# danilobellini/audiolazy

Measured on NVIDIA H100. Metric: samples/sec through 64-ch gammatone bank, higher is better.
Workload: dtype f64

## Files before the change

### audiolazy_b200/csrc/alz_capi.cu

```cuda
#pragma GCC visibility push(default)
#include "../../include/alz_b200.h"
#pragma GCC visibility pop
#include "alz_biquad.cuh"
#include "alz_generic.cuh"
#include "alz_lane_tma.cuh"
#include "alz_plan.h"

#include <algorithm>
#include <cctype>
#include <cmath>
#include <cstring>
#include <map>
#include <thread>

#include <sys/mman.h>
#include <sys/syscall.h>
#include <unistd.h>

static std::mutex g_host_mu;
static std::map<void*, size_t> g_host_allocs;

static_assert(ALZI_OK == ALZ_OK && ALZI_ERR_CUDA == ALZ_ERR_CUDA && ALZI_ERR_UNSUPPORTED == ALZ_ERR_UNSUPPORTED, "status codes");

static thread_local std::string g_err;
// ... 101 lines not shown
    const cuuint64_t ystr[3] = {(cuuint64_t)ta.T * 4, (cuuint64_t)ta.ys * 4, (cuuint64_t)ta.ysS * 4};
    const cuuint32_t ybox[4] = {32, 32, 1, 1};
    return enc(tmy, CU_TENSOR_MAP_DATA_TYPE_FLOAT32, 4, (void*)ta.y, ydims, ystr, ybox, estr, CU_TENSOR_MAP_INTERLEAVE_NONE,
               CU_TENSOR_MAP_SWIZZLE_128B, CU_TENSOR_MAP_L2_PROMOTION_NONE, CU_TENSOR_MAP_FLOAT_OOB_FILL_NONE) == CUDA_SUCCESS;
  }
  {
    const cuuint64_t dims[3] = {(cuuint64_t)ta.T, (cuuint64_t)ta.S, 1};
    const cuuint64_t strides[2] = {(cuuint64_t)ta.xs * 4, (cuuint64_t)ta.xs * 4};
    const cuuint32_t box[3] = {32, 32, 1};
    if (enc(tmx, CU_TENSOR_MAP_DATA_TYPE_FLOAT32, 3, (void*)ta.x, dims, strides, box, estr, CU_TENSOR_MAP_INTERLEAVE_NONE,
            CU_TENSOR_MAP_SWIZZLE_128B, CU_TENSOR_MAP_L2_PROMOTION_L2_128B, CU_TENSOR_MAP_FLOAT_OOB_FILL_NONE) != CUDA_SUCCESS)
      return false;
  }
  {
    const cuuint64_t dims[4] = {(cuuint64_t)ta.T, (cuuint64_t)ta.C, (cuuint64_t)ta.S, 1};
    const cuuint64_t strides[3] = {(cuuint64_t)ta.ys * 4, (cuuint64_t)ta.ysS * 4, (cuuint64_t)ta.ysS * 4};
    const cuuint32_t box[4] = {32, 1, 32, 1};
    if (enc(tmy, CU_TENSOR_MAP_DATA_TYPE_FLOAT32, 4, (void*)ta.y, dims, strides, box, estr, CU_TENSOR_MAP_INTERLEAVE_NONE,
            CU_TENSOR_MAP_SWIZZLE_128B, CU_TENSOR_MAP_L2_PROMOTION_NONE, CU_TENSOR_MAP_FLOAT_OOB_FILL_NONE) != CUDA_SUCCESS)
      return false;
  }
  return true;
}

static bool make_map_2d(const float* ptr, long long T, long long n_rows, long long stride, CUtensorMap* tm) {
  alz_encode_tiled_fn enc = get_encode_tiled();
  if (!enc || ((uintptr_t)ptr & 15) || (stride & 3) || T >= (1ll << 31) || n_rows >= (1ll << 31)) return false;
  const cuuint32_t estr[2] = {1, 1};
  const cuuint64_t dims[2] = {(cuuint64_t)T, (cuuint64_t)n_rows};
  const cuuint64_t strides[1] = {(cuuint64_t)stride * 4};
  const cuuint32_t box[2] = {32, 32};
  return enc(tm, CU_TENSOR_MAP_DATA_TYPE_FLOAT32, 2, (void*)ptr, dims, strides, box, estr, CU_TENSOR_MAP_INTERLEAVE_NONE,
             CU_TENSOR_MAP_SWIZZLE_128B, CU_TENSOR_MAP_L2_PROMOTION_L2_128B, CU_TENSOR_MAP_FLOAT_OOB_FILL_NONE) == CUDA_SUCCESS;
}

static int launch_biquad(const alz_plan* p, const AlzTileArgs& ta, cudaStream_t st) {
  if (p->NB0 == 8) {
    if (p->K == 1) return alzi_launch_headfir_k1(p, ta, st);
    if (p->K == 4) return alzi_launch_headfir_k4(p, ta, st);
    return fail(ALZ_ERR_UNSUPPORTED, "no head-FIR kernel for K=%d", p->K);
  }
  switch (p->K) {
    case 1: return alzi_launch_biquad_k1(p, ta, st);
    case 2: return alzi_launch_biquad_k2(p, ta, st);
    case 3: return alzi_launch_biquad_k3(p, ta, st);
    case 4: return alzi_launch_biquad_k4(p, ta, st);
    case 6: return alzi_launch_biquad_k6(p, ta, st);
    case 8: return alzi_launch_biquad_k8(p, ta, st);
  }
  return fail(ALZ_ERR_UNSUPPORTED, "no biquad kernel for K=%d", p->K);
}

static double probe_biquad(const alz_plan* p, const double* r64, const double* r32) {
  if (p->NB0 == 8) return p->K == 1 ? alzi_probe_headfir_k1(p, r64, r32) : alzi_probe_headfir_k4(p, r64, r32);
  switch (p->K) {
    case 1: return alzi_probe_biquad_k1(p, r64, r32);
    case 2: return alzi_probe_biquad_k2(p, r64, r32);
    case 3: return alzi_probe_biquad_k3(p, r64, r32);
    case 4: return alzi_probe_biquad_k4(p, r64, r32);
    case 6: return alzi_probe_biquad_k6(p, r64, r32);
    default: return alzi_probe_biquad_k8(p, r64, r32);
  }
}

static int launch_generic(const alz_plan* p, AlzTileArgs ta, cudaStream_t st, const double* tv = nullptr,
                          long long tv_stride = 0) {
  AlzGenericArgs ga{p->d_sec, p->d_tap_delay, p->d_coef, p->K, p->C, 0, tv, tv_stride};
  const long long groups = (ta.S + 31) / 32;
  CUtensorMap tmx, tmy;
  if (alzi_make_tensor_maps(ta, &tmx, &tmy))
    alz_generic_tma_kernel<<<dim3((unsigned)p->C, (unsigned)groups), 32, ALZ_TMA_SMEM, st>>>(ta, ga, tmx, tmy);
  else
    alz_generic_kernel<<<dim3((unsigned)p->C, (unsigned)groups), 32, ALZ_WARP_SMEM, st>>>(ta, ga);
  ALZ_CUDA(cudaGetLastError());
  g_launches.fetch_add(1, std::memory_order_relaxed);
  return ALZ_OK;
}

static const int kBiquadKs[] = {1, 2, 3, 4, 6, 8};

extern "C" {

const char* alz_last_error(void) { return g_err.c_str(); }
int32_t alz_abi_version(void) { return ALZ_ABI_VERSION; }
int64_t alz_launch_count(void) { return g_launches.load(); }

int32_t alz_device_count(void) {
  int n = 0;
  if (cudaGetDeviceCount(&n) != cudaSuccess) { cudaGetLastError(); return 0; }
  return n;
}

int32_t alz_set_device(int32_t device) {
  ALZ_CUDA(cudaSetDevice(device));
  return ALZ_OK;
}

int32_t alz_plan_create(const double* coef, const int32_t* desc, int32_t C, int32_t KM, alz_plan** out) {
  return alz_plan_create_ex(coef, desc, C, KM, 0, out);
}

int32_t alz_plan_create_ex(const double* coef, const int32_t* desc, int32_t C, int32_t KM, int32_t flags,
                           alz_plan** out) {
  if (!out) return fail(ALZ_ERR_INVALID, "out is null");
  *out = nullptr;
  if (!coef || !desc || C <= 0 || KM < 0) return fail(ALZ_ERR_INVALID, "bad plan arguments");
  const bool design_only = (flags & ALZ_PLAN_DESIGN_ONLY) != 0;
  int dev = -1;
  if (!design_only) ALZ_CUDA(cudaGetDevice(&dev));

  struct Sec { std::vector<double> b, a; };
  std::vector<std::vector<Sec>> secs(C);
  int Kmax = 0, nbmax = 1, namax = 1;
  for (int c = 0; c < C; ++c) {
    bool ended = false;
    for (int k = 0; k < KM; ++k) {
      const int32_t* d = desc + ((size_t)c * KM + k) * 3;
      const int nb = d[0], na = d[1];
      if (nb == 0) { ended = true; continue; }
      if (ended) return fail(ALZ_ERR_INVALID, "channel %d: section %d follows an absent section", c, k);
      if (nb < 0 || na < 1 || d[2] < 0) return fail(ALZ_ERR_INVALID, "channel %d section %d: bad descriptor", c, k);
      const double* b = coef + d[2];
      const double* a = b + nb;
      if (a[0] == 0.0) return fail(ALZ_ERR_ZERO_GAIN, "channel %d section %d: Invalid filter gain (a0 == 0)", c, k);
      Sec s;
      s.b.assign(b, b + nb);
      s.a.assign(a, a + na);
      const double a0 = a[0];
      if (a0 != 1.0) {
        for (auto& v : s.b) v /= a0;
        for (auto& v : s.a) v /= a0;
        s.a[0] = 1.0;
      }
      while (s.b.size() > 1 && s.b.back() == 0.0) s.b.pop_back();
      while (s.a.size() > 1 && s.a.back() == 0.0) s.a.pop_back();
      for (double v : s.b) if (!std::isfinite(v)) return fail(ALZ_ERR_INVALID, "non-finite coefficient");
      for (double v : s.a) if (!std::isfinite(v)) return fail(ALZ_ERR_INVALID, "non-finite coefficient");
      nbmax = std::max(nbmax, (int)s.b.size());
      namax = std::max(namax, (int)s.a.size());
      secs[c].push_back(std::move(s));
    }
    Kmax = std::max(Kmax, (int)secs[c].size());
  }
  if (Kmax == 0) Kmax = 1;

  alz_plan* p = new (std::nothrow) alz_plan();
  if (!p) return fail(ALZ_ERR_NOMEM, "out of host memory");
  p->C = C;
  p->device = dev;
  p->sequential = (flags & ALZ_PLAN_SEQUENTIAL) != 0;
  p->parallel_sum = (flags & ALZ_PLAN_PARALLEL) != 0;
  if (design_only || cudaDeviceGetAttribute(&p->sm_count, cudaDevAttrMultiProcessorCount, dev) != cudaSuccess || p->sm_count <= 0) {
    cudaGetLastError();
    p->sm_count = 132;
  }

  p->fr_desc.assign((size_t)C * Kmax * 3, 0);
  for (int c = 0; c < C; ++c)
    for (size_t k = 0; k < secs[c].size(); ++k) {
      int* d = &p->fr_desc[((size_t)c * Kmax + k) * 3];
      d[0] = (int)secs[c][k].b.size(); d[1] = (int)secs[c][k].a.size(); d[2] = (int)p->fr_coef.size();
      p->fr_coef.insert(p->fr_coef.end(), secs[c][k].b.begin(), secs[c][k].b.end());
      p->fr_coef.insert(p->fr_coef.end(), secs[c][k].a.begin(), secs[c][k].a.end());
    }
  p->fr_K = Kmax;

  int nb_first = 1, nb_rest = 1;
  for (int c = 0; c < C; ++c)
    for (size_t k = 0; k < secs[c].size(); ++k) {
      if (k == 0) nb_first = std::max(nb_first, (int)secs[c][k].b.size());
      else nb_rest = std::max(nb_rest, (int)secs[c][k].b.size());
    }
  const bool plain = nbmax <= 3 && namax <= 3 && Kmax <= 8;
  const bool headfir = !plain && namax <= 3 && nb_first <= 8 && nb_rest <= 3 && Kmax <= 4;
  const bool biquad = (plain || headfir) && !(flags & ALZ_PLAN_FORCE_GENERIC);
  if (biquad) {
    int K = 8;
    for (int kk : kBiquadKs) if (kk >= Kmax) { K = kk; break; }
    if (headfir) K = Kmax == 1 ? 1 : 4;
    p->kind = ALZ_KIND_BIQUAD;
    p->K = K;
    p->NB = headfir ? (nb_rest <= 1 ? 1 : 3) : nbmax;
    p->NB0 = headfir ? 8 : 0;
    p->xd = ALZ_H0(p->NB0); p->yd = 2;
    p->state_doubles = ALZ_STATE_SLOTS(K, p->NB0);
    bool monic = !p->parallel_sum;
    for (int c = 0; c < C && monic; ++c) {
      double g = 1.0;
      for (auto& s : secs[c]) {
        const double b0 = s.b[0];
        if (!(std::fabs(b0) > 1e-150 && std::fabs(b0) < 1e150)) { monic = false; break; }
        g *= b0;
        if (!(std::fabs(g) > 1e-250 && std::fabs(g) < 1e250)) { monic = false; break; }
      }
    }
    bool gain_in = monic && !env_int("ALZ_EXACT_GAIN", 0);
    for (int c = 0; c < C && gain_in; ++c) {
      double g = 1.0;
      for (auto& s : secs[c]) g *= s.b[0];
      if (!(std::fabs(g) > 1e-30 && std::fabs(g) < 1e30)) gain_in = false;
    }
    p->monic = monic ? (gain_in ? 2 : 1) : 0;
    p->fp64_ops = (monic ? K * (p->NB - 1 + 2) + (gain_in ? 0 : 1) : K * (p->NB + 2)) + (headfir ? 8 - p->NB : 0);
    if (!headfir && !env_int("ALZ_NO_ZMASK", 0)) {
      int zm = (1 << (2 * K)) - 1;
      for (int c = 0; c < C; ++c)
        for (size_t k = 0; k < secs[c].size(); ++k)
          for (int j = 1; j <= 2; ++j)
            if ((int)secs[c][k].b.size() > j && secs[c][k].b[j] != 0.0) zm &= ~(1 << (2 * (int)k + j - 1));
      p->zmask = zm;
      if (K == 4 && p->NB == 3 && (zm & ALZ_ZMASK_KLAPURI) == ALZ_ZMASK_KLAPURI) p->fp64_ops -= 6;
    }
    const int stride = ALZ_COEF_STRIDE(K, p->NB0), nval = ALZ_COEF_NVAL(K, p->NB0);
    std::vector<double> tab((size_t)C * stride, 0.0);
    p->sc.assign((size_t)C * (K + 1), 1.0);
    for (int c = 0; c < C; ++c) {
      double* rec = tab.data() + (size_t)c * stride;
      double g = 1.0, sc = 1.0;
      if (p->monic == 2) {
        double gg = 1.0;
        for (auto& s : secs[c]) gg *= s.b[0];
        sc = (double)(float)gg;
        p->sc[(size_t)c * (K + 1)] = sc;
      }
      for (int k = 0; k < K; ++k) {
        double b[8] = {1.0, 0, 0, 0, 0, 0, 0, 0}, a[3] = {1.0, 0.0, 0.0};
        if (k < (int)secs[c].size()) {
          const Sec& s = secs[c][k];
          b[0] = 0.0;
          for (size_t i = 0; i < s.b.size(); ++i) b[i] = s.b[i];
          for (size_t i = 0; i < s.a.size(); ++i) a[i] = s.a[i];
        }
        if (k == 0 && p->NB0 == 8)
          for (int j = 3; j < 8; ++j) rec[5 * K + 1 + (j - 3)] = monic ? b[j] / b[0] : b[j];
        if (monic) {
          rec[5 * k + 0] = 1.0;
          rec[5 * k + 1] = b[1] / b[0];
          rec[5 * k + 2] = b[2] / b[0];
          g *= b[0];
          sc /= b[0];
        } else {
          rec[5 * k + 0] = b[0];
          rec[5 * k + 1] = b[1];
          rec[5 * k + 2] = b[2];
        }
        rec[5 * k + 3] = -a[1];
        rec[5 * k + 4] = -a[2];
        p->sc[(size_t)c * (K + 1) + k + 1] = sc;
      }
      rec[5 * K] = monic ? g : 1.0;
    }
    p->tier.assign(C, 0);
    p->tier_err.assign(C, -1.0);
    p->tier_tol = env_double("ALZ_TIER_TOL", 2.5e-6);
    p->probe_len = std::max(64, env_int("ALZ_TIER_PROBE", 8192));
    const bool tiering = !(flags & ALZ_PLAN_EXACT) && !p->parallel_sum && !env_int("ALZ_NO_FP32_TIER", 0) && p->tier_tol > 0.0;
    std::vector<double> tab32((size_t)C * stride, 0.0);
    for (int c = 0; c < C; ++c) {
      const double* rec = tab.data() + (size_t)c * stride;
      float* r32 = reinterpret_cast<float*>(tab32.data() + (size_t)c * stride);
      bool representable = true;
      for (int i = 0; i < nval; ++i) {
        r32[i] = (float)rec[i];
        if (rec[i] != 0.0 && !(std::fabs(rec[i]) > 1e-30 && std::fabs(rec[i]) < 1e30)) representable = false;
      }
      if (tiering && representable) {
        p->tier_err[c] = probe_biquad(p, rec, tab32.data() + (size_t)c * stride);
        if (p->tier_err[c] <= p->tier_tol) { p->tier[c] = 1; ++p->n_fp32; }
      }
    }
    {
      std::vector<int> lst[2];
      const int order = env_int("ALZ_TIER_ORDER", 1);
      for (int c = 0; c < C; ++c) lst[order == 1 ? p->tier[c] : (order == 2 ? 1 - p->tier[c] : 0)].push_back(c);
      size_t i0 = 0, i1 = 0;
      p->pos_channel.clear();
      while (i0 < lst[0].size() || i1 < lst[1].size()) {
        const bool take0 = i1 >= lst[1].size() || (i0 < lst[0].size() && i0 * lst[1].size() <= i1 * lst[0].size());
        p->pos_channel.push_back(take0 ? lst[0][i0++] : lst[1][i1++]);
      }
    }
    p->h_tab.assign((size_t)C * stride, 0.0);
    for (int pos = 0; pos < C; ++pos) {
      const int c = p->pos_channel[pos];
      const std::vector<double>& src = p->tier[c] ? tab32 : tab;
      double* rec = p->h_tab.data() + (size_t)pos * stride;
      memcpy(rec, src.data() + (size_t)c * stride, (size_t)nval * sizeof(double));
      rec[ALZ_COEF_META(K, p->NB0)] = (double)(c + 65536 * p->tier[c]);
    }
    p->fp64_ops_exact = p->fp64_ops;
    p->coef_small = C * stride <= kCoefSmall;
    const int ncoef = p->coef_small ? kCoefSmall : kCoefLarge;
    const int per_launch = ncoef / stride;
    if (per_launch < 1) { alz_plan_destroy(p); return fail(ALZ_ERR_UNSUPPORTED, "coefficient record too large"); }
    for (int p0 = 0; p0 < C; p0 += per_launch) {
      const int npos = std::min(per_launch, C - p0);
      char* blk = (char*)calloc(1, 2 * sizeof(int) + (size_t)ncoef * sizeof(double));
      if (!blk) { alz_plan_destroy(p); return fail(ALZ_ERR_NOMEM, "out of host memory"); }
      reinterpret_cast<int*>(blk)[0] = stride;
      reinterpret_cast<int*>(blk)[1] = npos;
      memcpy(blk + 2 * sizeof(int), p->h_tab.data() + (size_t)p0 * stride, (size_t)npos * stride * sizeof(double));
      p->chunks.push_back({blk, npos});
    }
    p->tile_group = env_int("ALZ_TILE_GROUP", 2);
    if (p->tile_group != 1 && p->tile_group != 2 && p->tile_group != 4) p->tile_group = 2;
  } else if (Kmax == 1 && !(flags & ALZ_PLAN_FORCE_GENERIC) && C * 32 <= kCoefLarge && !env_int("ALZ_NO_WINDOW", 0)) {
    p->kind = ALZ_KIND_GENERIC;
    p->window = true;
    p->K = 1;
    p->NB = nbmax;
    p->monic = 0;
    int near_x = 0, near_y = 0, maxd_x = 0, maxd_y = 0;
    std::vector<int> far_x, far_y;
    for (int c = 0; c < C; ++c) {
      if (secs[c].empty()) continue;
      const Sec& s = secs[c][0];
      for (size_t d = 1; d < s.b.size(); ++d)
        if (s.b[d] != 0.0) {
          maxd_x = std::max(maxd_x, (int)d);
          if (d < 16) near_x = std::max(near_x, (int)d);
          else if (std::find(far_x.begin(), far_x.end(), (int)d) == far_x.end()) far_x.push_back((int)d);
        }
      for (size_t d = 1; d < s.a.size(); ++d)
        if (s.a[d] != 0.0) {
          maxd_y = std::max(maxd_y, (int)d);
          if (d < 16) near_y = std::max(near_y, (int)d);
          else if (std::find(far_y.begin(), far_y.end(), (int)d) == far_y.end()) far_y.push_back((int)d);
        }
    }
    std::sort(far_x.begin(), far_x.end());
    std::sort(far_y.begin(), far_y.end());
    auto slots_of = [](int nearest) { return nearest == 0 ? 0 : (nearest <= 3 ? 4 : 16); };
    auto pow2 = [](int n) { int q = 1; while (q < n) q <<= 1; return q; };
    p->win_mx = slots_of(near_x);
    p->win_my = slots_of(near_y);
    p->win_nfx = (int)far_x.size();
    p->win_nfy = (int)far_y.size();
    int slot = 1;
    p->win_xwin = slot; slot += p->win_mx ? p->win_mx - 1 : 0;
    p->win_ywin = slot; slot += p->win_my ? p->win_my - 1 : 0;
    if (!far_x.empty()) { p->win_xbase = slot; p->win_xmask = pow2(far_x.back() + 16) - 1; slot += p->win_xmask + 1; }
    if (!far_y.empty()) { p->win_ybase = slot; p->win_ymask = pow2(far_y.back() + 16) - 1; slot += p->win_ymask + 1; }
    p->xd = maxd_x; p->yd = maxd_y;
    p->state_doubles = slot;
    p->fp64_ops = 1 + (p->win_mx ? p->win_mx - 1 : 0) + (p->win_my ? p->win_my - 1 : 0) + p->win_nfx + p->win_nfy;
    p->win_far_delay = far_x;
    p->win_far_delay.insert(p->win_far_delay.end(), far_y.begin(), far_y.end());
    p->h_tab.assign((size_t)C * 32, 0.0);
    std::vector<double> fcoef(std::max<size_t>(1, p->win_far_delay.size()) * C, 0.0);
    for (int c = 0; c < C; ++c) {
      double* rec = p->h_tab.data() + (size_t)c * 32;
      if (secs[c].empty()) { rec[0] = 1.0; continue; }
      const Sec& s = secs[c][0];
      for (size_t d = 0; d < s.b.size() && d < 16; ++d) rec[d] = s.b[d];
      for (size_t d = 1; d < s.a.size() && d < 16; ++d) rec[16 + d - 1] = -s.a[d];
      for (size_t f = 0; f < far_x.size(); ++f) fcoef[f * C + c] = (size_t)far_x[f] < s.b.size() ? s.b[far_x[f]] : 0.0;
      for (size_t f = 0; f < far_y.size(); ++f) fcoef[(far_x.size() + f) * C + c] = (size_t)far_y[f] < s.a.size() ? -s.a[far_y[f]] : 0.0;
    }
    p->coef_small = C * 32 <= 64;
    p->win_block = calloc(1, alzi_window_block_bytes(p->coef_small));
    if (!p->win_block) { alz_plan_destroy(p); return fail(ALZ_ERR_NOMEM, "out of host memory"); }
    if (!design_only) {
      const size_t nf = std::max<size_t>(1, p->win_far_delay.size());
      std::vector<int> fd(nf, 16);
      std::copy(p->win_far_delay.begin(), p->win_far_delay.end(), fd.begin());
      cudaError_t e = cudaMalloc(&p->d_far_delay, nf * sizeof(int));
      if (e == cudaSuccess) e = cudaMemcpy(p->d_far_delay, fd.data(), nf * sizeof(int), cudaMemcpyHostToDevice);
      if (e == cudaSuccess) e = cudaMalloc(&p->d_far_coef, fcoef.size() * sizeof(double));
      if (e == cudaSuccess) e = cudaMemcpy(p->d_far_coef, fcoef.data(), fcoef.size() * sizeof(double), cudaMemcpyHostToDevice);
      if (e != cudaSuccess) { alz_plan_destroy(p); return fail(ALZ_ERR_CUDA, "plan upload failed: %s", cudaGetErrorString(e)); }
    }
    alzi_window_block_fill(p->win_block, p->coef_small, p->win_nfx, p->win_nfy, p->win_xbase, p->win_xmask, p->win_ybase,
                           p->win_ymask, p->win_xwin, p->win_ywin, C, p->d_far_delay, p->d_far_coef, p->h_tab.data());
  } else {
    const int K = Kmax;
    p->kind = ALZ_KIND_GENERIC;
    p->K = K;
    p->NB = nbmax;
    p->monic = 0;
    std::vector<int> tap_delay;
    std::vector<std::vector<double>> tap_coef;
    p->h_sec.resize(K);
    p->h_xlen.assign(K, 0);
    p->h_ylen.assign(K, 0);
    int slot = 1;
    int ops = 0, xdmax = 0, ydmax = 0;
    for (int k = 0; k < K; ++k) {
      size_t nb = 1, na = 1;
      for (int c = 0; c < C; ++c)
        if (k < (int)secs[c].size()) { nb = std::max(nb, secs[c][k].b.size()); na = std::max(na, secs[c][k].a.size()); }
      AlzGenSection gs{};
      gs.num_begin = (int)tap_delay.size();
      for (size_t d = 0; d < nb; ++d) {
        std::vector<double> col(C, 0.0);
        bool any = false;
        for (int c = 0; c < C; ++c) {
          double v;
          if (k < (int)secs[c].size()) v = d < secs[c][k].b.size() ? secs[c][k].b[d] : 0.0;
          else v = d == 0 ? 1.0 : 0.0;
          col[c] = v;
          any = any || v != 0.0;
        }
        if (any || d == 0) { tap_delay.push_back((int)d); tap_coef.push_back(std::move(col)); p->h_tap_is_den.push_back(0); }
      }
      gs.nnum = (int)tap_delay.size() - gs.num_begin;
      gs.den_begin = (int)tap_delay.size();
      for (size_t d = 1; d < na; ++d) {
        std::vector<double> col(C, 0.0);
        bool any = false;
        for (int c = 0; c < C; ++c) {
          double v = (k < (int)secs[c].size() && d < secs[c][k].a.size()) ? -secs[c][k].a[d] : 0.0;
          col[c] = v;
          any = any || v != 0.0;
        }
        if (any) { tap_delay.push_back((int)d); tap_coef.push_back(std::move(col)); p->h_tap_is_den.push_back(1); }
      }
      gs.nden = (int)tap_delay.size() - gs.den_begin;
      const int xlen = (int)nb - 1, ylen = (int)na - 1;
      auto pow2 = [](int n) { int q = 1; while (q < n) q <<= 1; return q; };
      if (xlen > 0) { gs.xbase = slot; gs.xmask = pow2(xlen) - 1; slot += gs.xmask + 1; } else { gs.xbase = 0; gs.xmask = -1; }
      if (ylen > 0) { gs.ybase = slot; gs.ymask = pow2(ylen) - 1; slot += gs.ymask + 1; } else { gs.ybase = 0; gs.ymask = -1; }
      p->h_sec[k] = gs;
      p->h_xlen[k] = xlen;
      p->h_ylen[k] = ylen;
      xdmax = std::max(xdmax, xlen);
      ydmax = std::max(ydmax, ylen);
      ops += gs.nnum + gs.nden;
    }
    p->xd = xdmax; p->yd = ydmax;
    p->state_doubles = slot;
    p->fp64_ops = ops;
    const size_t ntaps = tap_delay.size();
    p->h_tap_delay = tap_delay;
    std::vector<double> tab(ntaps * C);
    for (size_t t = 0; t < ntaps; ++t) memcpy(&tab[t * C], tap_coef[t].data(), C * sizeof(double));
    cudaError_t e = design_only ? cudaSuccess : cudaMalloc(&p->d_coef, tab.size() * sizeof(double));
    if (design_only) { *out = p; return ALZ_OK; }
    if (e == cudaSuccess) e = cudaMemcpy(p->d_coef, tab.data(), tab.size() * sizeof(double), cudaMemcpyHostToDevice);
    if (e == cudaSuccess) e = cudaMalloc(&p->d_sec, K * sizeof(AlzGenSection));
    if (e == cudaSuccess) e = cudaMemcpy(p->d_sec, p->h_sec.data(), K * sizeof(AlzGenSection), cudaMemcpyHostToDevice);
    if (e == cudaSuccess) e = cudaMalloc(&p->d_tap_delay, ntaps * sizeof(int));
    if (e == cudaSuccess) e = cudaMemcpy(p->d_tap_delay, tap_delay.data(), ntaps * sizeof(int), cudaMemcpyHostToDevice);
    if (e != cudaSuccess) { alz_plan_destroy(p); return fail(ALZ_ERR_CUDA, "plan upload failed: %s", cudaGetErrorString(e)); }
  }
  *out = p;
  return ALZ_OK;
}

void alz_plan_destroy(alz_plan* p) {
  if (!p) return;
  if (p->device < 0) {
    for (auto& ch : p->chunks) free(ch.block);
    free(p->win_block);
    delete p;
    return;
  }
  int cur = 0;
  cudaGetDevice(&cur);
  cudaSetDevice(p->device);
  if (p->pipe.ready) {
    for (int i = 0; i < AlzHostPipe::NBUF; ++i) {
      if (p->pipe.stream[i]) { cudaStreamSynchronize(p->pipe.stream[i]); cudaStreamDestroy(p->pipe.stream[i]); }
      if (p->pipe.done[i]) cudaEventDestroy(p->pipe.done[i]);
      cudaFree(p->pipe.dx[i]);
      cudaFree(p->pipe.dy[i]);
      cudaFree(p->pipe.dst[i]);
      cudaFree(p->pipe.des[i]);
    }
  }
  for (auto& ch : p->chunks) free(ch.block);
  for (auto& e : p->m_cache) { cudaFree(e.M); cudaEventDestroy(e.ready); }
  free(p->win_block);
  cudaFree(p->d_far_delay);
  cudaFree(p->d_far_coef);
  cudaFree(p->d_coef);
  cudaFree(p->d_sec);
  cudaFree(p->d_tap_delay);
  cudaFree(p->d_fr_coef);
  cudaFree(p->d_fr_desc);
  cudaSetDevice(cur);
  cudaGetLastError();
  delete p;
}

int32_t alz_plan_info_get(const alz_plan* p, alz_plan_info* out) {
  if (!p || !out) return fail(ALZ_ERR_INVALID, "null argument");
  memset(out, 0, sizeof *out);
  out->abi_version = ALZ_ABI_VERSION;
  out->kind = p->kind;
  out->n_channels = p->C;
  out->n_sections = p->K;
  out->num_taps = p->NB0 ? p->NB0 : p->NB;
  out->monic = p->monic;
  out->state_doubles = p->state_doubles;
  out->fp64_ops = p->fp64_ops;
  out->device = p->device;
  out->n_fp32_channels = p->n_fp32;
  out->tier_tol_e9 = (int32_t)std::min(2.0e9, p->tier_tol * 1e9 + 0.5);
  return ALZ_OK;
}

int32_t alz_plan_tiers(const alz_plan* p, int32_t* tier, double* probe_err, int32_t cap) {
  if (!p) return fail(ALZ_ERR_INVALID, "plan is null");
  for (int c = 0; c < p->C && c < cap; ++c) {
    const bool have = c < (int)p->tier.size();
    if (tier) tier[c] = have ? p->tier[c] : 0;
    if (probe_err) probe_err[c] = have ? p->tier_err[c] : -1.0;
  }
  return p->C;
}

int64_t alz_plan_state_doubles(const alz_plan* p, int64_t S) {
  if (!p || S < 0) return fail(ALZ_ERR_INVALID, "bad argument");
  return (int64_t)p->state_doubles * S * p->C;
}

int32_t alz_plan_history(const alz_plan* p, int32_t* xd, int32_t* yd) {
  if (!p || !xd || !yd) return fail(ALZ_ERR_INVALID, "null argument");
  *xd = p->xd;
  *yd = p->yd;
  return ALZ_OK;
}

static __global__ void alz_state_fill_kernel(double* state, const double* proto, long long R, int C, int slots) {
  const long long i = (long long)blockIdx.x * blockDim.x + threadIdx.x;
  if (i >= R * slots) return;
  const long long slot = i / R, r = i - slot * R, S = R / C;
  state[i] = proto[slot * C + (int)(r / S)];
}

int32_t alz_state_init(const alz_plan* p, double* state, int64_t S, const double* xinit, const double* yinit,
                       void* cuda_stream) {
  if (!p || S < 0) return fail(ALZ_ERR_INVALID, "bad argument");
  if (p->device < 0) return fail(ALZ_ERR_CUDA, "design-only plan: no device");
  if (S == 0) return ALZ_OK;
  if (!state) return fail(ALZ_ERR_INVALID, "state is null");
  cudaStream_t st = (cudaStream_t)cuda_stream;
  const long long R = (long long)S * p->C;
  const size_t bytes = (size_t)p->state_doubles * R * sizeof(double);
  if (!xinit && !yinit) {
    ALZ_CUDA(cudaMemsetAsync(state, 0, bytes, st));
    return ALZ_OK;
  }
  const int C = p->C, K = p->K, slots = p->state_doubles;
  std::vector<double> proto((size_t)slots * C, 0.0);
  if (p->kind == ALZ_KIND_BIQUAD) {
    for (int c = 0; c < C; ++c)
      for (int k = 0; k < K; ++k) {
        const double sc_in = p->sc[(size_t)c * (K + 1) + k], sc_out = p->sc[(size_t)c * (K + 1) + k + 1];
        const int base = ALZ_STATE_BASE(k, p->NB0);
        const int nx = k == 0 ? ALZ_H0(p->NB0) : 2;
        for (int j = 0; j < nx; ++j) {
          const double xv = xinit ? xinit[((size_t)c * K + k) * p->xd + j] : 0.0;
          proto[(size_t)(base + j) * C + c] = (p->monic == 2 && k == 0) ? (double)((float)xv * (float)sc_in) : xv * sc_in;
        }
        for (int j = 0; j < 2; ++j) {
          const double yv = yinit ? yinit[((size_t)c * K + k) * 2 + j] : 0.0;
          proto[(size_t)(base + nx + j) * C + c] = yv * sc_out;
        }
      }
  } else if (p->window) {
    for (int c = 0; c < C; ++c) {
      for (int j = 0; j < p->xd; ++j) {
        const double xv = xinit ? xinit[(size_t)c * p->xd + j] : 0.0;
        if (j + 1 < p->win_mx) proto[(size_t)(p->win_xwin + j) * C + c] = xv;
        if (p->win_xmask >= 0) proto[(size_t)(p->win_xbase + ((-(j + 1)) & p->win_xmask)) * C + c] = xv;
      }
      for (int j = 0; j < p->yd; ++j) {
        const double yv = yinit ? yinit[(size_t)c * p->yd + j] : 0.0;
        if (j + 1 < p->win_my) proto[(size_t)(p->win_ywin + j) * C + c] = yv;
        if (p->win_ymask >= 0) proto[(size_t)(p->win_ybase + ((-(j + 1)) & p->win_ymask)) * C + c] = yv;
      }
    }
  } else {
    for (int c = 0; c < C; ++c)
      for (int k = 0; k < K; ++k) {
        const AlzGenSection& gs = p->h_sec[k];
        for (int j = 0; j < p->h_xlen[k]; ++j) {
          const double xv = xinit ? xinit[((size_t)c * K + k) * p->xd + j] : 0.0;
          proto[(size_t)(gs.xbase + ((-(j + 1)) & gs.xmask)) * C + c] = xv;
        }
        for (int j = 0; j < p->h_ylen[k]; ++j) {
          const double yv = yinit ? yinit[((size_t)c * K + k) * p->yd + j] : 0.0;
          proto[(size_t)(gs.ybase + ((-(j + 1)) & gs.ymask)) * C + c] = yv;
        }
      }
  }
  double* d_proto = nullptr;
  ALZ_CUDA(cudaMallocAsync((void**)&d_proto, proto.size() * sizeof(double), st));
  ALZ_CUDA(cudaMemcpyAsync(d_proto, proto.data(), proto.size() * sizeof(double), cudaMemcpyHostToDevice, st));
  const long long n = R * slots;
  alz_state_fill_kernel<<<(unsigned)((n + 255) / 256), 256, 0, st>>>(state, d_proto, R, C, slots);
  ALZ_CUDA(cudaGetLastError());
  g_launches.fetch_add(1, std::memory_order_relaxed);
  ALZ_CUDA(cudaFreeAsync(d_proto, st));
  ALZ_CUDA(cudaStreamSynchronize(st));
  return ALZ_OK;
}

static int apply_launch(const alz_plan* p, AlzTileArgs ta, double* state, long long sstride, cudaStream_t st,
                        const double* tv, long long tv_stride) {
  ta.state = state;
  ta.sstride = sstride;
  if (p->kind == ALZ_KIND_BIQUAD) return launch_biquad(p, ta, st);
  if (p->window) return alzi_launch_window(p, ta, st);
  return launch_generic(p, ta, st, tv, tv_stride);
}

// ... 791 lines not shown
```

### audiolazy_b200/csrc/alz_lane_tma.cuh

```cuda
#pragma once
#include <cuda.h>
#include "alz_lane.cuh"

#define ALZ_TMA_TILE_BYTES 4096
#define ALZ_TMA_MAX_GROUP 4
#define ALZ_TMA_SMEM_FOR(ng) (((ng) < 2 ? 2 : (ng)) * ALZ_TMA_TILE_BYTES + 8 * ALZ_TMA_MAX_GROUP)
#define ALZ_TMA_SMEM ALZ_TMA_SMEM_FOR(2)

__device__ __forceinline__ unsigned alz_smem_u32(const void* p) { return (unsigned)__cvta_generic_to_shared(p); }

__device__ __forceinline__ void alz_mbar_init(unsigned mbar, unsigned count) {
  asm volatile("mbarrier.init.shared::cta.b64 [%0], %1;\n" ::"r"(mbar), "r"(count) : "memory");
}
__device__ __forceinline__ void alz_mbar_expect_tx(unsigned mbar, unsigned bytes) {
  asm volatile("mbarrier.arrive.expect_tx.shared::cta.b64 _, [%0], %1;\n" ::"r"(mbar), "r"(bytes) : "memory");
}
__device__ __forceinline__ void alz_mbar_wait(unsigned mbar, unsigned parity) {
  asm volatile(
      "{\n"
      ".reg .pred p;\n"
      "ALZ_WAIT:\n"
      "mbarrier.try_wait.parity.shared::cta.b64 p, [%0], %1;\n"
      "@p bra ALZ_DONE;\n"
      "bra ALZ_WAIT;\n"
      "ALZ_DONE:\n"
      "}\n" ::"r"(mbar), "r"(parity) : "memory");
}
__device__ __forceinline__ void alz_tma_load_2d(unsigned dst, const CUtensorMap* map, int c0, int c1, unsigned mbar) {
  asm volatile("cp.async.bulk.tensor.2d.shared::cluster.global.mbarrier::complete_tx::bytes [%0], [%1, {%2, %3}], [%4];\n"
               ::"r"(dst), "l"(reinterpret_cast<unsigned long long>(map)), "r"(c0), "r"(c1), "r"(mbar) : "memory");
}
__device__ __forceinline__ void alz_tma_store_3d(const CUtensorMap* map, int c0, int c1, int c2, unsigned src) {
  asm volatile("cp.async.bulk.tensor.3d.global.shared::cta.bulk_group [%0, {%1, %2, %3}], [%4];\n"
               ::"l"(reinterpret_cast<unsigned long long>(map)), "r"(c0), "r"(c1), "r"(c2), "r"(src) : "memory");
}
__device__ __forceinline__ void alz_tma_store_2d(const CUtensorMap* map, int c0, int c1, unsigned src) {
  asm volatile("cp.async.bulk.tensor.2d.global.shared::cta.bulk_group [%0, {%1, %2}], [%3];\n"
               ::"l"(reinterpret_cast<unsigned long long>(map)), "r"(c0), "r"(c1), "r"(src) : "memory");
}
__device__ __forceinline__ void alz_tma_load_3d(unsigned dst, const CUtensorMap* map, int c0, int c1, int c2, unsigned mbar) {
  asm volatile("cp.async.bulk.tensor.3d.shared::cluster.global.mbarrier::complete_tx::bytes [%0], [%1, {%2, %3, %4}], [%5];\n"
               ::"r"(dst), "l"(reinterpret_cast<unsigned long long>(map)), "r"(c0), "r"(c1), "r"(c2), "r"(mbar) : "memory");
}
__device__ __forceinline__ void alz_tma_store_4d(const CUtensorMap* map, int c0, int c1, int c2, int c3, unsigned src) {
  asm volatile("cp.async.bulk.tensor.4d.global.shared::cta.bulk_group [%0, {%1, %2, %3, %4}], [%5];\n"
               ::"l"(reinterpret_cast<unsigned long long>(map)), "r"(c0), "r"(c1), "r"(c2), "r"(c3), "r"(src) : "memory");
}
__device__ __forceinline__ void alz_bulk_commit() { asm volatile("cp.async.bulk.commit_group;\n" ::: "memory"); }
__device__ __forceinline__ void alz_bulk_wait_read0() { asm volatile("cp.async.bulk.wait_group.read 0;\n" ::: "memory"); }
__device__ __forceinline__ void alz_bulk_wait0() { asm volatile("cp.async.bulk.wait_group 0;\n" ::: "memory"); }
__device__ __forceinline__ void alz_fence_async_smem() { asm volatile("fence.proxy.async.shared::cta;\n" ::: "memory"); }

struct AlzStoreY {
  static constexpr bool active = false;
};
struct AlzEnvelopePost {
  static constexpr bool active = true;
  double env;
  float* out;
  double* st;
  int left;
  __device__ __forceinline__ void load(const AlzTileArgs& a, int c, long long row, unsigned chunk, long long r, long long tbeg) {
    st = a.env_state + r;
    env = __ldcg(st);
    const unsigned pos = (unsigned)a.env_phase + (unsigned)tbeg + chunk * (unsigned)a.T;
    const unsigned q = pos / (unsigned)a.env_decim;
    out = a.env_out + (row * a.C + c) * a.env_es + q;
    left = a.env_store ? a.env_decim - (int)(pos - q * (unsigned)a.env_decim) : 0x7fffffff;
  }
  __device__ __forceinline__ void tile(const AlzTileArgs& a, const float* row, int swz, int nvalid, bool valid) {
    for (int j = 0; j < nvalid; ++j) {
      const float y = row[(((j >> 2) ^ swz) << 2) | (j & 3)];
      const double r = a.env_mode == 0 ? (double)fabsf(y) : (double)y * (double)y;
      env = fma(a.env_R, env, a.env_g * r);
      if (--left == 0) {
        if (valid) *out =(float)(a.env_mode == 2 ? sqrt(env) : env);
        ++out;
        left = a.env_decim;
      }
    }
  }
  __device__ __forceinline__ void store() { *st = env; }
};

template <class Core, class Post = AlzStoreY, class CoreArgs>
__device__ __forceinline__ void alz_run_warp_tma(const AlzTileArgs& a, const CoreArgs& ca, const CUtensorMap* tmx,
                                                 const CUtensorMap* tmy, unsigned char* smem) {
  const int lane = threadIdx.x;
  const int c_local = blockIdx.x;
  const int c = ca.channel(c_local);
  int group = blockIdx.y, seg = 0;
  long long tbeg = 0, tlen = a.T;
  unsigned* flag = nullptr;
  if (a.nseg > 1) {
    unsigned ticket = 0;
    if (lane == 0) ticket = atomicAdd(a.sync + c_local, 1u);
    ticket = __shfl_sync(0xffffffffu, ticket, 0);
    seg = (int)(ticket / (unsigned)a.groups);
    group = (int)(ticket - (unsigned)seg * (unsigned)a.groups);
    tbeg = (long long)seg * a.seg_len;
    tlen = a.T - tbeg < a.seg_len ? a.T - tbeg : a.seg_len;
    flag = a.sync + gridDim.x + (size_t)c_local * a.groups + group;
    if (seg > 0) {
      unsigned done;
      do {
        asm volatile("ld.acquire.gpu.global.u32 %0, [%1];\n" : "=r"(done) : "l"(flag) : "memory");
      } while (done < (unsigned)seg);
    }
  }
  const long long s0 = (long long)group * 32;
  const long long s = s0 + lane;
  const bool valid = s < a.S;
  const long long r = (long long)c * a.Stot + (valid ? s : a.S - 1);
  int ld1 = (int)s0, ld2 = 0, st1 = c, st2 = (int)s0, st3 = 0;
  if (a.vP > 0) {
    ld2 = (int)(s0 / a.vP);
    ld1 = (int)(s0 - (long long)ld2 * a.vP);
    st1 = ld1; st2 = c; st3 = ld2;
  }

  const int NG = a.paired < 2 ? 1 : a.paired;
  const int nbuf = NG < 2 ? 2 : NG;
  const unsigned tile0 = alz_smem_u32(smem);
  const unsigned mbar0 = tile0 + nbuf * ALZ_TMA_TILE_BYTES;
  if (lane == 0) {
    for (int j = 0; j < nbuf; ++j) alz_mbar_init(mbar0 + 8 * j, 1);
    asm volatile("fence.mbarrier_init.release.cluster;\n" ::: "memory");
  }
  __syncwarp();

  Core core;
  core.load(a, ca, r, c_local, valid);
  Post post;
  if constexpr (Post::active) {
    if (a.vP > 0) post.load(a, c, ld2, (unsigned)(ld1 + lane), r, tbeg);
    else post.load(a, c, valid ? s : a.S - 1, 0u, r, tbeg);
  }

  const int ntiles = (int)((tlen + ALZ_TT - 1) / ALZ_TT);
  const int nfull = (int)(tlen / ALZ_TT);
  const int tb = (int)tbeg;
  const int swz = lane & 7;
  float* const myrow = reinterpret_cast<float*>(smem) + lane * 32;
  const bool tail_by_lanes = (a.T & 3) != 0 && nfull < ntiles;
  int last_buf = 0;

  const int lg = NG >= 4 ? 2 : (NG >= 2 ? 1 : 0);
  if (lane == 0 && NG == 1) {
    alz_mbar_expect_tx(mbar0, ALZ_TMA_TILE_BYTES);
    alz_tma_load_3d(tile0, tmx, tb, ld1, ld2, mbar0);
  }
  for (int i = 0; i < ntiles; ++i) {
    const int j = NG == 1 ? (i & 1) : (i & (NG - 1));
    const int t0 = i * ALZ_TT;
    const bool skip_load = (a.exp & 1) && i >= NG;
    if (lane == 0 && !skip_load) {
      if (NG == 1) {
        if (i + 1 < ntiles) {
          if (i >= 1) alz_bulk_wait_read0();
          alz_mbar_expect_tx(mbar0 + 8 * (j ^ 1), ALZ_TMA_TILE_BYTES);
          alz_tma_load_3d(tile0 + (j ^ 1) * ALZ_TMA_TILE_BYTES, tmx, tb + t0 + ALZ_TT, ld1, ld2, mbar0 + 8 * (j ^ 1));
        }
      } else if (j == 0) {
        if (i > 0) alz_bulk_wait_read0();
        const int n = ntiles - i < NG ? ntiles - i : NG;
        for (int jj = 0; jj < n; ++jj) {
          alz_mbar_expect_tx(mbar0 + 8 * jj, ALZ_TMA_TILE_BYTES);
          alz_tma_load_3d(tile0 + jj * ALZ_TMA_TILE_BYTES, tmx, tb + t0 + jj * ALZ_TT, ld1, ld2, mbar0 + 8 * jj);
        }
      }
    }
    if (!((a.exp & 1) && i >= (NG == 1 ? 2 : NG)))
      alz_mbar_wait(mbar0 + 8 * j, (NG == 1 ? (i >> 1) : (i >> lg)) & 1);
    const int nvalid = i < nfull ? ALZ_TT : (int)(tlen - t0);
    core.tile(myrow + j * (ALZ_TMA_TILE_BYTES / 4), swz, nvalid, t0);
    if constexpr (Post::active) post.tile(a, myrow + j * (ALZ_TMA_TILE_BYTES / 4), swz, nvalid, valid);
    alz_fence_async_smem();
    __syncwarp();
    const bool last = i + 1 == ntiles;
    if (lane == 0 && !(a.exp & 2) && !Post::active) {
      if (NG == 1) {
        if (!(tail_by_lanes && last)) alz_tma_store_4d(tmy, tb + t0, st1, st2, st3, tile0 + j * ALZ_TMA_TILE_BYTES);
        alz_bulk_commit();
      } else if (j == NG - 1 || last) {
        for (int jj = 0; jj <= j; ++jj)
          if (!(tail_by_lanes && last && jj == j))
            alz_tma_store_4d(tmy, tb + t0 - (j - jj) * ALZ_TT, st1, st2, st3, tile0 + jj * ALZ_TMA_TILE_BYTES);
        alz_bulk_commit();
      }
    }
    last_buf = j;
  }
  if (tail_by_lanes && valid && !Post::active) {
    const int i = ntiles - 1, t0 = i * ALZ_TT, nvalid = (int)(tlen - t0);
    const float* src = myrow + last_buf * (ALZ_TMA_TILE_BYTES / 4);
    float* dst = a.y + s * a.ysS + (long long)c * a.ys + tbeg + t0;
    for (int j = 0; j < nvalid; ++j) dst[j] = src[(((j >> 2) ^ swz) << 2) | (j & 3)];
  }
  if (lane == 0) alz_bulk_wait0();
  if (valid) core.store(a, r, tlen);
  if constexpr (Post::active) { if (valid) post.store(); }
  if (flag != nullptr && seg + 1 < a.nseg) {
    __threadfence();
    __syncwarp();
    if (lane == 0) asm volatile("st.release.gpu.global.u32 [%0], %1;\n" ::"l"(flag), "r"((unsigned)(seg + 1)) : "memory");
  }
}
```

### audiolazy_b200/csrc/alz_launch.cuh

```cuda
#pragma once
#include <algorithm>
#include <cmath>
#include <cstring>

#include "alz_biquad.cuh"
#include "alz_lane_tma.cuh"
#include "alz_plan.h"

static const int kCoefSmall = 512, kCoefLarge = 3584;
static const int kWarpsPerSm = 22;
static const int kWarpsPerSmTma = 24;

template <int K, int NB, int MONIC, int NCOEF, int NB0, int ZMASK>
__global__ void __launch_bounds__(32, kWarpsPerSm)
alz_biquad_kernel(const __grid_constant__ AlzTileArgs a, const __grid_constant__ AlzBiquadArgs<NCOEF> ca) {
  extern __shared__ __align__(16) float alz_smem[];
  if (ca.tier(blockIdx.x) == 0) alz_run_warp<AlzBiquadCore<K, NB, MONIC, NB0, ZMASK, double>>(a, ca, alz_smem);
  else alz_run_warp<AlzBiquadCore<K, NB, MONIC, NB0, ZMASK, float>>(a, ca, alz_smem);
}

template <int K, int NB, int MONIC, int NCOEF, int NB0, int ZMASK>
__global__ void __launch_bounds__(32, kWarpsPerSmTma)
alz_biquad_tma_kernel(const __grid_constant__ AlzTileArgs a, const __grid_constant__ AlzBiquadArgs<NCOEF> ca,
                      const __grid_constant__ CUtensorMap tmx, const __grid_constant__ CUtensorMap tmy) {
  extern __shared__ __align__(1024) unsigned char alz_smem_tma[];
  if (ca.tier(blockIdx.x) == 0)
    alz_run_warp_tma<AlzBiquadCore<K, NB, MONIC, NB0, ZMASK, double>>(a, ca, &tmx, &tmy, alz_smem_tma);
  else
    alz_run_warp_tma<AlzBiquadCore<K, NB, MONIC, NB0, ZMASK, float>>(a, ca, &tmx, &tmy, alz_smem_tma);
}

template <int K, int NB, int MONIC, int NCOEF, int NB0, int ZMASK>
__global__ void __launch_bounds__(32, kWarpsPerSmTma)
alz_biquad_envelope_kernel(const __grid_constant__ AlzTileArgs a, const __grid_constant__ AlzBiquadArgs<NCOEF> ca,
                           const __grid_constant__ CUtensorMap tmx, const __grid_constant__ CUtensorMap tmy) {
  extern __shared__ __align__(1024) unsigned char alz_smem_tma[];
  if (ca.tier(blockIdx.x) == 0)
    alz_run_warp_tma<AlzBiquadCore<K, NB, MONIC, NB0, ZMASK, double>, AlzEnvelopePost>(a, ca, &tmx, &tmy, alz_smem_tma);
  else
    alz_run_warp_tma<AlzBiquadCore<K, NB, MONIC, NB0, ZMASK, float>, AlzEnvelopePost>(a, ca, &tmx, &tmy, alz_smem_tma);
}

template <int K, int NB, int NB0, int ZMASK>
static int launch_envelope_t(const alz_plan* p, AlzTileArgs ta, cudaStream_t st) {
  if (p->coef_small || p->chunks.size() != 1)
    return alzi_fail(ALZI_ERR_UNSUPPORTED, "envelope consumer: gammatone-bank plans only");
  CUtensorMap tmx, tmy;
  if (!alzi_make_tensor_maps(ta, &tmx, &tmy)) return alzi_fail(ALZI_ERR_UNSUPPORTED, "envelope consumer needs 16-byte aligned x rows");
  const long long groups = (ta.S + 31) / 32;
  ta.paired = (long long)p->chunks[0].npos * groups >= (long long)p->sm_count * kWarpsPerSmTma ? 2 : 1;
  ta.groups = (int)groups;
  void* args[4] = {(void*)&ta, p->chunks[0].block, (void*)&tmx, (void*)&tmy};
  const void* kern = p->monic == 2 ? (const void*)alz_biquad_envelope_kernel<K, NB, 2, kCoefLarge, NB0, ZMASK>
                   : p->monic == 1 ? (const void*)alz_biquad_envelope_kernel<K, NB, 1, kCoefLarge, NB0, ZMASK>
                                   : (const void*)alz_biquad_envelope_kernel<K, NB, 0, kCoefLarge, NB0, ZMASK>;
  ALZ_CUDA(cudaLaunchKernel(kern, dim3((unsigned)p->chunks[0].npos, (unsigned)groups), dim3(32), args, ALZ_TMA_SMEM_FOR(ta.paired), st));
  ALZ_CUDA(cudaGetLastError());
  alzi_launches.fetch_add(1, std::memory_order_relaxed);
  return ALZI_OK;
}

template <int K, int NB, int MONIC, int NCOEF, int NB0, int ZMASK>
static int launch_biquad_chunk(const alz_plan* p, AlzTileArgs ta, const void* block, int npos, cudaStream_t st) {
  const long long groups = (ta.S + 31) / 32;
  CUtensorMap tmx, tmy;
  if (alzi_make_tensor_maps(ta, &tmx, &tmy)) {
    const long long warps = (long long)npos * groups;
    int ng = warps >= (long long)p->sm_count * kWarpsPerSmTma ? p->tile_group : 1;
    ng = alzi_env_int("ALZ_TMA_PAIRED", ng);
    if (ng != 2 && ng != 4) ng = 1;
    ta.paired = ng;
    ta.exp |= alzi_env_int("ALZ_EXP", 0);
    const size_t smem = ALZ_TMA_SMEM_FOR(ng);
    const long long per_sm = std::min<long long>(kWarpsPerSmTma, (228 * 1024) / (long long)(smem + 1024));
    const long long slots = (long long)p->sm_count * per_sm;
    long long nseg = 1;
    if (ta.vP == 0 && warps > slots && warps < 8 * slots && ta.T >= 2048 && !alzi_env_int("ALZ_NO_SEGMENT", 0)) {
      const long long waves = std::max(1, alzi_env_int("ALZ_SEG_WAVES", 16)), min_len = std::max(32, alzi_env_int("ALZ_SEG_MIN", 1024));
      nseg = std::min((waves * slots + warps - 1) / warps, ta.T / min_len);
      const long long quantum = 32ll * ng;
      const long long len = ((ta.T + nseg - 1) / nseg + quantum - 1) / quantum * quantum;
      nseg = (ta.T + len - 1) / len;
      if (nseg > 1 && groups * nseg <= 65535) {
        const size_t words = (size_t)npos + (size_t)npos * groups;
        unsigned* sync = nullptr;
        alzi_keep_async_pool();
        ALZ_CUDA(cudaMallocAsync(&sync, words * 4, st));
        if (cudaMemsetAsync(sync, 0, words * 4, st) != cudaSuccess) {
          cudaFreeAsync(sync, st);
          ALZ_CUDA(cudaGetLastError());
        }
        ta.nseg = (int)nseg; ta.seg_len = len; ta.sync = sync;
      } else {
        nseg = 1;
      }
    }
    ta.groups = (int)groups;
    auto kern = alz_biquad_tma_kernel<K, NB, MONIC, NCOEF, NB0, ZMASK>;
    if (smem > 48 * 1024) return alzi_fail(ALZI_ERR_UNSUPPORTED, "tile group too large");
    void* args[4] = {(void*)&ta, const_cast<void*>(block), (void*)&tmx, (void*)&tmy};
    const cudaError_t e = cudaLaunchKernel((const void*)kern, dim3((unsigned)npos, (unsigned)(groups * nseg)), dim3(32), args, smem, st);
    if (ta.sync) cudaFreeAsync(ta.sync, st);
    ALZ_CUDA(e);
  } else {
    if (ta.exp & 2) ta.y = nullptr;
    auto kern = alz_biquad_kernel<K, NB, MONIC, NCOEF, NB0, ZMASK>;
    void* args[2] = {(void*)&ta, const_cast<void*>(block)};
    ALZ_CUDA(cudaLaunchKernel((const void*)kern, dim3((unsigned)npos, (unsigned)groups), dim3(32), args, ALZ_WARP_SMEM, st));
  }
  ALZ_CUDA(cudaGetLastError());
  alzi_launches.fetch_add(1, std::memory_order_relaxed);
  return ALZI_OK;
}

template <int K, int NB, int MONIC, int NB0, int ZMASK>
static int launch_biquad_t(const alz_plan* p, const AlzTileArgs& ta, cudaStream_t st) {
  for (const auto& ch : p->chunks) {
    const int rc = p->coef_small ? launch_biquad_chunk<K, NB, MONIC, kCoefSmall, NB0, ZMASK>(p, ta, ch.block, ch.npos, st)
                                 : launch_biquad_chunk<K, NB, MONIC, kCoefLarge, NB0, ZMASK>(p, ta, ch.block, ch.npos, st);
    if (rc != ALZI_OK) return rc;
  }
  return ALZI_OK;
}

template <int K, int NB, int NB0, int ZMASK = 0>
static int launch_biquad_nb(const alz_plan* p, const AlzTileArgs& ta, cudaStream_t st) {
  if (p->monic == 2) return launch_biquad_t<K, NB, 2, NB0, ZMASK>(p, ta, st);
  if (p->monic == 1) return launch_biquad_t<K, NB, 1, NB0, ZMASK>(p, ta, st);
  return launch_biquad_t<K, NB, 0, NB0, ZMASK>(p, ta, st);
}

template <int K>
static int launch_biquad_k(const alz_plan* p, const AlzTileArgs& ta, cudaStream_t st) {
  switch (p->NB) {
    case 1: return launch_biquad_nb<K, 1, 0>(p, ta, st);
    case 2: return launch_biquad_nb<K, 2, 0>(p, ta, st);
    default:
      if constexpr (K == 4) {
        if ((p->zmask & ALZ_ZMASK_KLAPURI) == ALZ_ZMASK_KLAPURI) return launch_biquad_nb<4, 3, 0, ALZ_ZMASK_KLAPURI>(p, ta, st);
      }
      return launch_biquad_nb<K, 3, 0>(p, ta, st);
  }
}

template <int K>
static int launch_headfir_k(const alz_plan* p, const AlzTileArgs& ta, cudaStream_t st) {
  if constexpr (K == 1) return launch_biquad_nb<1, 1, 8>(p, ta, st);
  else {
    if (p->NB <= 1) return launch_biquad_nb<K, 1, 8>(p, ta, st);
    return launch_biquad_nb<K, 3, 8>(p, ta, st);
  }
}

static inline float alzi_probe_noise(unsigned& s) {
  s = s * 1664525u + 1013904223u;
  return (float)((double)(s >> 8) * (2.0 / 16777216.0) - 1.0);
}

template <int K, int NB, int MONIC, int NB0, int ZMASK>
static double probe_biquad_t(const double* rec64, const double* rec32, int n) {
  double worst = 0.0;
  for (int sig = 0; sig < 5; ++sig) {
    AlzBiquadCore<K, NB, MONIC, NB0, ZMASK, double> c64;
    AlzBiquadCore<K, NB, MONIC, NB0, ZMASK, float> c32;
    c64.load_coef(rec64); c64.zero_state();
    c32.load_coef(rec32); c32.zero_state();
    unsigned seed = 12345u;
    double peak = 0.0, err = 0.0;
    for (int i = 0; i < n; ++i) {
      const float nyq = (i & 1) ? -1.0f : 1.0f;
      const float x = sig == 0 ? alzi_probe_noise(seed) : sig == 1 ? 1.0f : sig == 2 ? (i == 0 ? 1.0f : 0.0f)
                      : sig == 3 ? 0.5f * alzi_probe_noise(seed) + 0.5f * nyq : nyq;
      float y64, y32;
      if (i < 2) { y64 = c64.step_explicit(c64.widen(x)); y32 = c32.step_explicit(c32.widen(x)); }
      else { y64 = c64.step_alias(c64.widen(x)); y32 = c32.step_alias(c32.widen(x)); }
      peak = std::max(peak, std::fabs((double)y64));
      const double d = std::fabs((double)y32 - (double)y64);
      err = std::max(err, d == d ? d : 1e300);
    }
    if (peak > 0.0) worst = std::max(worst, err / peak);
    else if (err > 0.0) worst = 1e300;
  }
  return worst;
}

template <int K, int NB, int NB0, int ZMASK = 0>
static double probe_biquad_nb(const alz_plan* p, const double* r64, const double* r32, int n) {
  if (p->monic == 2) return probe_biquad_t<K, NB, 2, NB0, ZMASK>(r64, r32, n);
  if (p->monic == 1) return probe_biquad_t<K, NB, 1, NB0, ZMASK>(r64, r32, n);
  return probe_biquad_t<K, NB, 0, NB0, ZMASK>(r64, r32, n);
}

template <int K>
static double probe_biquad_k(const alz_plan* p, const double* r64, const double* r32) {
  const int n = p->probe_len;
  switch (p->NB) {
    case 1: return probe_biquad_nb<K, 1, 0>(p, r64, r32, n);
    case 2: return probe_biquad_nb<K, 2, 0>(p, r64, r32, n);
    default:
      if constexpr (K == 4) {
        if ((p->zmask & ALZ_ZMASK_KLAPURI) == ALZ_ZMASK_KLAPURI) return probe_biquad_nb<4, 3, 0, ALZ_ZMASK_KLAPURI>(p, r64, r32, n);
      }
      return probe_biquad_nb<K, 3, 0>(p, r64, r32, n);
  }
}

template <int K>
static double probe_headfir_k(const alz_plan* p, const double* r64, const double* r32) {
  if constexpr (K == 1) return probe_biquad_nb<1, 1, 8>(p, r64, r32, p->probe_len);
  else {
    if (p->NB <= 1) return probe_biquad_nb<K, 1, 8>(p, r64, r32, p->probe_len);
    return probe_biquad_nb<K, 3, 8>(p, r64, r32, p->probe_len);
  }
}
```

Baseline: 8.331 billion.

## Add L2 cache hints to TMA loads/stores and default to 4-tile groups

Adds createpolicy-based L2 eviction hints: input tiles are loaded evict_last and output tiles stored evict_first when grouping two or more tiles with no vP path. The default tile group rises from 2 to 4, capped at 2 when vP>0. The upper bound on warps for time segmentation is removed, so segmentation can also kick in for very large grids. These aim to keep the shared input resident in L2 and to deepen TMA batching, at the cost of more shared memory per warp and possibly lower occupancy.

Result: faster. 9.038 billion (median of 6 runs) (+8.5%).

```diff
diff --git a/audiolazy_b200/csrc/alz_capi.cu b/audiolazy_b200/csrc/alz_capi.cu
--- a/audiolazy_b200/csrc/alz_capi.cu
+++ b/audiolazy_b200/csrc/alz_capi.cu
@@ -427,8 +427,8 @@
       memcpy(blk + 2 * sizeof(int), p->h_tab.data() + (size_t)p0 * stride, (size_t)npos * stride * sizeof(double));
       p->chunks.push_back({blk, npos});
     }
-    p->tile_group = env_int("ALZ_TILE_GROUP", 2);
-    if (p->tile_group != 1 && p->tile_group != 2 && p->tile_group != 4) p->tile_group = 2;
+    p->tile_group = env_int("ALZ_TILE_GROUP", 4);
+    if (p->tile_group != 1 && p->tile_group != 2 && p->tile_group != 4) p->tile_group = 4;
   } else if (Kmax == 1 && !(flags & ALZ_PLAN_FORCE_GENERIC) && C * 32 <= kCoefLarge && !env_int("ALZ_NO_WINDOW", 0)) {
     p->kind = ALZ_KIND_GENERIC;
     p->window = true;
diff --git a/audiolazy_b200/csrc/alz_lane_tma.cuh b/audiolazy_b200/csrc/alz_lane_tma.cuh
--- a/audiolazy_b200/csrc/alz_lane_tma.cuh
+++ b/audiolazy_b200/csrc/alz_lane_tma.cuh
@@ -38,6 +38,16 @@
   asm volatile("cp.async.bulk.tensor.2d.global.shared::cta.bulk_group [%0, {%1, %2}], [%3];\n"
                ::"l"(reinterpret_cast<unsigned long long>(map)), "r"(c0), "r"(c1), "r"(src) : "memory");
 }
+__device__ __forceinline__ unsigned long long alz_policy_evict_first() {
+  unsigned long long p;
+  asm volatile("createpolicy.fractional.L2::evict_first.b64 %0, 1.0;\n" : "=l"(p));
+  return p;
+}
+__device__ __forceinline__ unsigned long long alz_policy_evict_last() {
+  unsigned long long p;
+  asm volatile("createpolicy.fractional.L2::evict_last.b64 %0, 1.0;\n" : "=l"(p));
+  return p;
+}
 __device__ __forceinline__ void alz_tma_load_3d(unsigned dst, const CUtensorMap* map, int c0, int c1, int c2, unsigned mbar) {
   asm volatile("cp.async.bulk.tensor.3d.shared::cluster.global.mbarrier::complete_tx::bytes [%0], [%1, {%2, %3, %4}], [%5];\n"
                ::"r"(dst), "l"(reinterpret_cast<unsigned long long>(map)), "r"(c0), "r"(c1), "r"(c2), "r"(mbar) : "memory");
@@ -45,6 +55,19 @@
 __device__ __forceinline__ void alz_tma_store_4d(const CUtensorMap* map, int c0, int c1, int c2, int c3, unsigned src) {
   asm volatile("cp.async.bulk.tensor.4d.global.shared::cta.bulk_group [%0, {%1, %2, %3, %4}], [%5];\n"
                ::"l"(reinterpret_cast<unsigned long long>(map)), "r"(c0), "r"(c1), "r"(c2), "r"(c3), "r"(src) : "memory");
+}
+__device__ __forceinline__ void alz_tma_load_3d(unsigned dst, const CUtensorMap* map, int c0, int c1, int c2, unsigned mbar,
+                                                unsigned long long pol) {
+  asm volatile("cp.async.bulk.tensor.3d.shared::cluster.global.mbarrier::complete_tx::bytes.L2::cache_hint"
+               " [%0], [%1, {%2, %3, %4}], [%5], %6;\n"
+               ::"r"(dst), "l"(reinterpret_cast<unsigned long long>(map)), "r"(c0), "r"(c1), "r"(c2), "r"(mbar), "l"(pol)
+               : "memory");
+}
+__device__ __forceinline__ void alz_tma_store_4d(const CUtensorMap* map, int c0, int c1, int c2, int c3, unsigned src,
+                                                 unsigned long long pol) {
+  asm volatile("cp.async.bulk.tensor.4d.global.shared::cta.bulk_group.L2::cache_hint [%0, {%1, %2, %3, %4}], [%5], %6;\n"
+               ::"l"(reinterpret_cast<unsigned long long>(map)), "r"(c0), "r"(c1), "r"(c2), "r"(c3), "r"(src), "l"(pol)
+               : "memory");
 }
 __device__ __forceinline__ void alz_bulk_commit() { asm volatile("cp.async.bulk.commit_group;\n" ::: "memory"); }
 __device__ __forceinline__ void alz_bulk_wait_read0() { asm volatile("cp.async.bulk.wait_group.read 0;\n" ::: "memory"); }
@@ -146,9 +169,19 @@
   int last_buf = 0;
 
   const int lg = NG >= 4 ? 2 : (NG >= 2 ? 1 : 0);
+  const bool hint = NG >= 2 && a.vP == 0;
+  const unsigned long long pol_x = hint ? alz_policy_evict_last() : 0ull, pol_y = hint ? alz_policy_evict_first() : 0ull;
+  auto load_x = [&](unsigned dst, int t, unsigned mbar) {
+    if (hint) alz_tma_load_3d(dst, tmx, t, ld1, ld2, mbar, pol_x);
+    else alz_tma_load_3d(dst, tmx, t, ld1, ld2, mbar);
+  };
+  auto store_y = [&](int t, unsigned src) {
+    if (hint) alz_tma_store_4d(tmy, t, st1, st2, st3, src, pol_y);
+    else alz_tma_store_4d(tmy, t, st1, st2, st3, src);
+  };
   if (lane == 0 && NG == 1) {
     alz_mbar_expect_tx(mbar0, ALZ_TMA_TILE_BYTES);
-    alz_tma_load_3d(tile0, tmx, tb, ld1, ld2, mbar0);
+    load_x(tile0, tb, mbar0);
   }
   for (int i = 0; i < ntiles; ++i) {
     const int j = NG == 1 ? (i & 1) : (i & (NG - 1));
@@ -159,14 +192,14 @@
         if (i + 1 < ntiles) {
           if (i >= 1) alz_bulk_wait_read0();
           alz_mbar_expect_tx(mbar0 + 8 * (j ^ 1), ALZ_TMA_TILE_BYTES);
-          alz_tma_load_3d(tile0 + (j ^ 1) * ALZ_TMA_TILE_BYTES, tmx, tb + t0 + ALZ_TT, ld1, ld2, mbar0 + 8 * (j ^ 1));
+          load_x(tile0 + (j ^ 1) * ALZ_TMA_TILE_BYTES, tb + t0 + ALZ_TT, mbar0 + 8 * (j ^ 1));
         }
       } else if (j == 0) {
         if (i > 0) alz_bulk_wait_read0();
         const int n = ntiles - i < NG ? ntiles - i : NG;
         for (int jj = 0; jj < n; ++jj) {
           alz_mbar_expect_tx(mbar0 + 8 * jj, ALZ_TMA_TILE_BYTES);
-          alz_tma_load_3d(tile0 + jj * ALZ_TMA_TILE_BYTES, tmx, tb + t0 + jj * ALZ_TT, ld1, ld2, mbar0 + 8 * jj);
+          load_x(tile0 + jj * ALZ_TMA_TILE_BYTES, tb + t0 + jj * ALZ_TT, mbar0 + 8 * jj);
         }
       }
     }
@@ -180,12 +213,12 @@
     const bool last = i + 1 == ntiles;
     if (lane == 0 && !(a.exp & 2) && !Post::active) {
       if (NG == 1) {
-        if (!(tail_by_lanes && last)) alz_tma_store_4d(tmy, tb + t0, st1, st2, st3, tile0 + j * ALZ_TMA_TILE_BYTES);
+        if (!(tail_by_lanes && last)) store_y(tb + t0, tile0 + j * ALZ_TMA_TILE_BYTES);
         alz_bulk_commit();
       } else if (j == NG - 1 || last) {
         for (int jj = 0; jj <= j; ++jj)
           if (!(tail_by_lanes && last && jj == j))
-            alz_tma_store_4d(tmy, tb + t0 - (j - jj) * ALZ_TT, st1, st2, st3, tile0 + jj * ALZ_TMA_TILE_BYTES);
+            store_y(tb + t0 - (j - jj) * ALZ_TT, tile0 + jj * ALZ_TMA_TILE_BYTES);
         alz_bulk_commit();
       }
     }
diff --git a/audiolazy_b200/csrc/alz_launch.cuh b/audiolazy_b200/csrc/alz_launch.cuh
--- a/audiolazy_b200/csrc/alz_launch.cuh
+++ b/audiolazy_b200/csrc/alz_launch.cuh
@@ -66,7 +66,7 @@
   CUtensorMap tmx, tmy;
   if (alzi_make_tensor_maps(ta, &tmx, &tmy)) {
     const long long warps = (long long)npos * groups;
-    int ng = warps >= (long long)p->sm_count * kWarpsPerSmTma ? p->tile_group : 1;
+    int ng = warps >= (long long)p->sm_count * kWarpsPerSmTma ? (ta.vP > 0 ? std::min(p->tile_group, 2) : p->tile_group) : 1;
     ng = alzi_env_int("ALZ_TMA_PAIRED", ng);
     if (ng != 2 && ng != 4) ng = 1;
     ta.paired = ng;
@@ -75,7 +75,7 @@
     const long long per_sm = std::min<long long>(kWarpsPerSmTma, (228 * 1024) / (long long)(smem + 1024));
     const long long slots = (long long)p->sm_count * per_sm;
     long long nseg = 1;
-    if (ta.vP == 0 && warps > slots && warps < 8 * slots && ta.T >= 2048 && !alzi_env_int("ALZ_NO_SEGMENT", 0)) {
+    if (ta.vP == 0 && warps > slots && ta.T >= 2048 && !alzi_env_int("ALZ_NO_SEGMENT", 0)) {
       const long long waves = std::max(1, alzi_env_int("ALZ_SEG_WAVES", 16)), min_len = std::max(32, alzi_env_int("ALZ_SEG_MIN", 1024));
       nseg = std::min((waves * slots + warps - 1) / warps, ta.T / min_len);
       const long long quantum = 32ll * ng;
```
